# Girjoaba/simplex_method_gpu

Hardware: AMD Instinct MI355X
Metric: simplex iterations/sec on dense m=4096 n=16384 fp64; achieved HBM GB/s (higher is better)
Workload: dtype f64

## Files before the change

### include/simplex.h

```cpp
#ifndef SIMPLEX_MI355X_H
#define SIMPLEX_MI355X_H

#include <stdint.h>

#ifdef __cplusplus
extern "C" {
#endif

#define SPX_ABI_VERSION 8

#define SPX_STATUS_MAX_ITER       0
#define SPX_STATUS_OPTIMUM_FOUND  1
#define SPX_STATUS_UNBOUNDED      2
#define SPX_STATUS_THETA_OVERFLOW 3
#define SPX_STATUS_INFEASIBLE     4

#define SPX_OK             0
#define SPX_ERR_ARG       -1
#define SPX_ERR_HIP       -2
#define SPX_ERR_OOM       -3
#define SPX_ERR_RCCL      -4
#define SPX_ERR_STATE     -5
#define SPX_ERR_NO_DEVICE -6
#define SPX_ERR_SINGULAR  -7
// ... 143 lines not shown

int spx_solve(spx_ctx* ctx, int64_t max_iter, double* z, int64_t* b_ixs,
              double* x_b, int32_t* status, int64_t* pivots);

int spx_iterate(spx_ctx* ctx, int64_t k, int32_t* status, int64_t* pivots);

int spx_price(spx_ctx* ctx, int64_t* p, double* min_e, int32_t* optimal);
int spx_pivot(spx_ctx* ctx, int64_t* q, int32_t* status);

int spx_get_state(spx_ctx* ctx, double* x_b, int64_t* b_ixs, double* y,
                  double* c_b, double* binv_rowmajor, int32_t* status,
                  int64_t* pivots);

int spx_reduced_costs(spx_ctx* ctx, double* e);

int spx_objective(spx_ctx* ctx, double* z);

int spx_get_trace(spx_ctx* ctx, int64_t* p, int64_t* q, int64_t cap, int64_t* count);

int spx_get_weights(spx_ctx* ctx, double* w);

int spx_kernel_times(spx_ctx* ctx, double* price_ms, int64_t* price_launches,
                     double* update_ms, int64_t* update_launches);

int spx_pbox_vtb_times(spx_ctx* ctx, double* ms, int64_t* launches);

int spx_pbox_wexact_times(spx_ctx* ctx, double* ms, int64_t* launches);

int spx_ranging_times(spx_ctx* ctx, double ms[2], int64_t launches[2]);

int spx_pass_times(spx_ctx* ctx, double out[3], int64_t* passes);

#define SPX_PHASES 18
int spx_phase_times(spx_ctx* ctx, double out[SPX_PHASES]);

int spx_fold_times(spx_ctx* ctx, uint64_t* out, int64_t cap, int64_t* count);

int spx_wg_times(spx_ctx* ctx, uint64_t* out, int64_t cap, int64_t* count);

#define SPX_LOOP_FIELDS 7
int spx_loop_times(spx_ctx* ctx, double out[SPX_LOOP_FIELDS], int64_t* passes);

int spx_info(spx_ctx* ctx, int64_t* m, int64_t* n, int64_t* ld,
             int64_t* local_nonbasic, double* bytes_price, double* bytes_update);

#define SPX_CONFIG_FIELDS 17
int spx_config(spx_ctx* ctx, int32_t out[SPX_CONFIG_FIELDS]);

#define SPX_LOOP_LAYOUT_FIELDS 8
int spx_loop_layout(spx_ctx* ctx, int32_t out[SPX_LOOP_LAYOUT_FIELDS]);

int spx_ftran_cols(spx_ctx* ctx, int32_t* cols);

#define SPX_DISPATCH_FIELDS 12
int spx_dispatch_stats(spx_ctx* ctx, int64_t out[SPX_DISPATCH_FIELDS]);

int spx_prepare(spx_ctx* ctx);

int spx_shard_range(int64_t m, int64_t n, int32_t rank, int32_t nranks, int64_t out[4]);
int spx_minloc_merge(const double* vals, const int64_t* idx, int32_t count,
                     double* best_val, int64_t* best_idx);

const char* spx_last_error(void);
const char* spx_status_string(int32_t status);
int spx_abi_version(void);

#ifdef __cplusplus
}
#endif
#endif
```

### simplex_method_gpu_amd/__init__.py

```python
from __future__ import annotations

import ctypes
from dataclasses import dataclass
from enum import IntEnum
from typing import NamedTuple

import numpy as np

from ._lib import SimplexError, SpxOpts, check, load

__all__ = ["SolveStatus", "SolveResult", "Context", "solve", "read_lp", "comm_unique_id",
           "shard_range", "minloc_merge", "group_iterate", "group_sync", "check_ranks",
           "SimplexError", "FLAG_TIMING", "RATIO_REFERENCE", "RATIO_GUARDED", "RATIO_HARRIS",
           "PRICING_DANTZIG", "PRICING_DEVEX", "PRICING_STEEPEST", "ALGO_PRIMAL", "ALGO_DUAL",
           "DUAL_PRICING_DANTZIG", "DUAL_PRICING_STEEPEST", "FLAG_DUAL_STEEPEST",
           "DUAL_RATIO_TEXTBOOK", "DUAL_RATIO_LONG_STEP", "FLAG_DUAL_LONG_STEP", "ALGO_PRIMAL_BOX",
           "FLAG_PRIMAL_PHASE1", "PRIMAL_PRICING_DANTZIG", "PRIMAL_PRICING_STEEPEST", "FLAG_PRIMAL_STEEPEST",
           "PRIMAL_WEIGHTS_REFERENCE", "PRIMAL_WEIGHTS_EXACT", "FLAG_PRIMAL_EXACT_WEIGHTS",
           "CostRanging", "RhsRanging"]

FLAG_TIMING = 1
FLAG_STAMPS = 2
FLAG_GLOBAL_Y = 4
FLAG_ROW_SHARD = 8
# ... 457 lines not shown
        per = 4 * min(g, 4096) + 4 * min(gp, 4096) + 3
        out = np.zeros(2 * per, dtype=np.uint64)
        cnt = ctypes.c_int64()
        check(self._L.spx_wg_times(self._h, _ptr(out), out.size, ctypes.byref(cnt)))
        res = []
        for par in range(2):
            b = out[par * per: (par + 1) * per]
            nu, npr = 4 * min(g, 4096), 4 * min(gp, 4096)
            res.append({"ftran": b[:nu].reshape(-1, 4), "price": b[nu: nu + npr].reshape(-1, 4),
                        "tail": int(b[nu + npr]), "mark": int(b[nu + npr + 1]), "book": int(b[nu + npr + 2])})
        return res

    def fold_times(self):
        out = np.zeros(8 * 1024, dtype=np.uint64)
        cnt = ctypes.c_int64()
        check(self._L.spx_fold_times(self._h, _ptr(out), out.size, ctypes.byref(cnt)))
        return out.reshape(1024, 8)

    def phase_times(self):
        out = (ctypes.c_double * 18)()
        check(self._L.spx_phase_times(self._h, out))
        return {"price_body_us": out[0], "price_tail_us": out[1],
                "update_body_us": out[2], "update_tail_us": out[3],
                "tail_partials_us": out[4], "tail_sy_us": out[5], "tail_blocksum_us": out[6],
                "tail_bookkeeping_us": out[7], "update_prologue_us": out[9], "update_drain_us": out[10],
                "price_prologue_us": out[11], "price_drain_us": out[12],
                "upd_wg0_us": [round(out[13 + k], 2) for k in range(5)]}

    def loop_times(self):
        out, n = (ctypes.c_double * 7)(), ctypes.c_int64()
        check(self._L.spx_loop_times(self._h, out, ctypes.byref(n)))
        return {"loop_ms": out[0], "loop_passes": int(out[1]), "price_us": out[2], "ftran_us": out[3],
                "tail_us": out[4], "clock_passes": n.value, "fold_ms": out[5], "folds": int(out[6])}

    def pass_times(self):
        out, n = (ctypes.c_double * 3)(), ctypes.c_int64()
        check(self._L.spx_pass_times(self._h, out, ctypes.byref(n)))
        return {"price_ms": out[0], "price_minloc_ms": out[1], "update_ms": out[2], "passes": n.value}

    def info(self):
        m, n, ld, nb = ctypes.c_int64(), ctypes.c_int64(), ctypes.c_int64(), ctypes.c_int64()
        bp, bu = ctypes.c_double(), ctypes.c_double()
        check(self._L.spx_info(self._h, ctypes.byref(m), ctypes.byref(n), ctypes.byref(ld), ctypes.byref(nb),
                               ctypes.byref(bp), ctypes.byref(bu)))
        return {"m": m.value, "n": n.value, "ld": ld.value, "local_nonbasic": nb.value,
                "bytes_price": bp.value, "bytes_update": bu.value}


    def ftran_cols(self) -> int:
        v = ctypes.c_int32()
        check(self._L.spx_ftran_cols(self._h, ctypes.byref(v)))
        return v.value

    def dispatch_stats(self):
        out = (ctypes.c_int64 * 12)()
        check(self._L.spx_dispatch_stats(self._h, out))
        keys = ("eager_passes", "graph_launches", "graph_passes", "persistent_launches", "persistent_passes",
                "folds", "window_pos", "window", "persist_fallbacks", "graph_builds", "dw_anchors", "dw_carry")
        return dict(zip(keys, list(out)))

    def config(self):
        out = (ctypes.c_int32 * 17)()
        check(self._L.spx_config(self._h, out))
        keys = ("window", "price_block", "price_grid", "price_lds", "update_block", "update_rows", "update_grid",
                "graph_batch", "persistent", "loop_block", "tableau", "loop_grid", "defer_tail", "compact_fold",
                "ftran_rows_per_wave", "mbox_fused", "compact_price")
        cfg = dict(zip(keys, list(out)))
        cfg["dw_carry"] = self.dispatch_stats()["dw_carry"]
        cfg["dual_pricing"] = self._dual_pricing
        cfg["primal_pricing"] = self._primal_pricing
        cfg["dual_ratio"] = self._dual_ratio
        cfg["primal_weights"] = self._primal_weights
        return cfg

    def loop_layout(self):
        out = (ctypes.c_int32 * 8)()
        check(self._L.spx_loop_layout(self._h, out))
        keys = ("dual_price_lds", "dual_update_lds", "dual_se_update_lds", "dual_se_rho_lds", "pbox_price_lds",
                "pbox_update_lds", "pbox_se_lds_vecs", "slack_unit")
        return dict(zip(keys, list(out)))


def solve(A_cols, b, c, max_iter: int = (1 << 62), eps: float = 1e-7, device: int = -1,
          algorithm: int = ALGO_PRIMAL) -> SolveResult:
    with Context(A_cols, b, c, eps=eps, device=device, algorithm=algorithm) as ctx:
        return ctx.solve(max_iter)
```

### simplex_method_gpu_amd/_lib.py

```python
from __future__ import annotations

import ctypes
import os

_HERE = os.path.dirname(os.path.abspath(__file__))
LIB_PATH = os.environ.get("SPX_LIB") or os.path.join(_HERE, "libsimplex.so")

_d, _i32, _i64, _u64, _p = ctypes.c_double, ctypes.c_int32, ctypes.c_int64, ctypes.c_uint64, ctypes.c_void_p
_pp = ctypes.POINTER(ctypes.c_void_p)


class SpxOpts(ctypes.Structure):
    _fields_ = [
        ("eps", ctypes.c_double),
        ("device", ctypes.c_int32),
        ("rank", ctypes.c_int32),
        ("nranks", ctypes.c_int32),
        ("graph_batch", ctypes.c_int32),
        ("price_block", ctypes.c_int32),
        ("update_rows", ctypes.c_int32),
        ("price_grid", ctypes.c_int32),
        ("flags", ctypes.c_int32),
        ("update_block", ctypes.c_int32),
        ("window", ctypes.c_int32),
        ("ratio_test", ctypes.c_int32),
        ("refactor_every", ctypes.c_int32),
        ("piv_tol", ctypes.c_double),
        ("feas_tol", ctypes.c_double),
        ("pricing", ctypes.c_int32),
        ("loop_block", ctypes.c_int32),
        ("trace_cap", ctypes.c_int32),
        ("algorithm", ctypes.c_int32),
    ]


SIGNATURES = {
    "spx_default_opts": (None, [ctypes.POINTER(SpxOpts)]),
    "spx_create": (ctypes.c_int, [_pp, _i64, _i64, _p, _p, _p, ctypes.POINTER(SpxOpts)]),
    "spx_create_generated": (ctypes.c_int, [_pp, _i64, _i64, _u64, ctypes.POINTER(SpxOpts)]),
    "spx_destroy": (None, [_p]),
    "spx_comm_unique_id": (ctypes.c_int, [_p]),
    "spx_attach_comm": (ctypes.c_int, [_p, _p]),
    "spx_comm_info": (ctypes.c_int, [_p, _p, _p]),
    "spx_mbox_export": (ctypes.c_int, [_p, _p]),
    "spx_ftran_cols": (ctypes.c_int, [_p, _p]),
    "spx_mbox_attach": (ctypes.c_int, [_p, _p]),
    "spx_reset": (ctypes.c_int, [_p]),
    "spx_reinvert": (ctypes.c_int, [_p]),
    "spx_set_basis": (ctypes.c_int, [_p, _p]),
    "spx_set_algorithm": (ctypes.c_int, [_p, _i32]),
    "spx_set_rhs": (ctypes.c_int, [_p, _p]),
    "spx_set_bounds": (ctypes.c_int, [_p, _p]),
    "spx_get_bounds": (ctypes.c_int, [_p, _p]),
    "spx_set_bounds_lu": (ctypes.c_int, [_p, _p, _p]),
    "spx_get_bounds_lu": (ctypes.c_int, [_p, _p, _p]),
    "spx_get_primal": (ctypes.c_int, [_p, _p, _p]),
    "spx_set_dual_pricing": (ctypes.c_int, [_p, _i32]),
    "spx_get_dual_weights": (ctypes.c_int, [_p, _p]),
    "spx_set_dual_ratio": (ctypes.c_int, [_p, _i32]),
    "spx_set_primal_pricing": (ctypes.c_int, [_p, _i32]),
    "spx_get_primal_weights": (ctypes.c_int, [_p, _p]),
    "spx_get_dual_flips": (ctypes.c_int, [_p, _p]),
    "spx_set_cost": (ctypes.c_int, [_p, _p]),
    "spx_get_primal_flips": (ctypes.c_int, [_p, _p]),
    "spx_pbox_vtb_times": (ctypes.c_int, [_p, _p, _p]),
    "spx_set_primal_weight_init": (ctypes.c_int, [_p, _i32]),
    "spx_refresh_primal_weights": (ctypes.c_int, [_p]),
    "spx_pbox_wexact_times": (ctypes.c_int, [_p, _p, _p]),
    "spx_ranging_cost": (ctypes.c_int, [_p, _p, _p, _p, _p]),
    "spx_ranging_rhs": (ctypes.c_int, [_p, _p, _p, _p, _p]),
    "spx_ranging_times": (ctypes.c_int, [_p, _p, _p]),
    "spx_group_iterate": (ctypes.c_int, [_p, _i32, _i64, _p, _p]),
    "spx_group_sync": (ctypes.c_int, [_p, _i32]),
    "spx_solve": (ctypes.c_int, [_p, _i64, _p, _p, _p, _p, _p]),
    "spx_iterate": (ctypes.c_int, [_p, _i64, _p, _p]),
    "spx_price": (ctypes.c_int, [_p, _p, _p, _p]),
    "spx_pivot": (ctypes.c_int, [_p, _p, _p]),
    "spx_dispatch_stats": (ctypes.c_int, [_p, _p]),
    "spx_prepare": (ctypes.c_int, [_p]),
    "spx_get_trace": (ctypes.c_int, [_p, _p, _p, _i64, _p]),
    "spx_get_weights": (ctypes.c_int, [_p, _p]),
    "spx_get_state": (ctypes.c_int, [_p, _p, _p, _p, _p, _p, _p, _p]),
    "spx_reduced_costs": (ctypes.c_int, [_p, _p]),
    "spx_objective": (ctypes.c_int, [_p, _p]),
    "spx_kernel_times": (ctypes.c_int, [_p, _p, _p, _p, _p]),
    "spx_pass_times": (ctypes.c_int, [_p, _p, _p]),
    "spx_info": (ctypes.c_int, [_p, _p, _p, _p, _p, _p, _p]),
    "spx_config": (ctypes.c_int, [_p, _p]),
    "spx_loop_layout": (ctypes.c_int, [_p, _p]),
    "spx_phase_times": (ctypes.c_int, [_p, _p]),
    "spx_wg_times": (ctypes.c_int, [_p, _p, _i64, _p]),
    "spx_fold_times": (ctypes.c_int, [_p, _p, _i64, _p]),
    "spx_loop_times": (ctypes.c_int, [_p, _p, _p]),
    "spx_shard_range": (ctypes.c_int, [_i64, _i64, _i32, _i32, _p]),
    "spx_minloc_merge": (ctypes.c_int, [_p, _p, _i32, _p, _p]),
    "spx_last_error": (ctypes.c_char_p, []),
    "spx_status_string": (ctypes.c_char_p, [_i32]),
    "spx_abi_version": (ctypes.c_int, []),
# ... 35 lines not shown
```

### simplex_method_gpu_amd/csrc/spx_api.cpp

```cpp
#include <algorithm>
#include <cmath>
#include <cstdarg>
#include <cstdio>
#include <cstdlib>
#include <cstring>
#include <string>
#include <vector>

#include "spx_ctx.h"
#include "spx_tableau.h"

using namespace spx;
using namespace spx_host;

namespace {

thread_local std::string g_err;

}

int spx_host::fail(int code, const char* fmt, ...) {
    char buf[512];
    va_list ap;
    va_start(ap, fmt);
    vsnprintf(buf, sizeof(buf), fmt, ap);
    va_end(ap);
    g_err = buf;
    return code;
}

namespace {

int64_t round_up(int64_t v, int64_t a) { return (v + a - 1) / a * a; }

void shard_range(int64_t m, int64_t n, int r, int G, int64_t out[4]) {
    const int64_t ns = n - m;
    const int64_t sb = (ns + G - 1) / G, kb = (m + G - 1) / G;
    out[0] = std::min<int64_t>(ns, (int64_t)r * sb);
    out[1] = std::min<int64_t>(ns, (int64_t)(r + 1) * sb);
    out[2] = ns + std::min<int64_t>(m, (int64_t)r * kb);
    out[3] = ns + std::min<int64_t>(m, (int64_t)(r + 1) * kb);
}

}

extern "C" {

void spx_default_opts(spx_opts* o) {
    if (!o) return;
    std::memset(o, 0, sizeof(*o));
    o->eps = 1e-7;
    o->device = -1;
    o->rank = 0;
    o->nranks = 1;
    o->graph_batch = 0;
    o->ratio_test = SPX_RATIO_REFERENCE;
    o->refactor_every = 0;
    o->piv_tol = 1e-9;
    o->feas_tol = 1e-9;
    o->pricing = SPX_PRICING_DANTZIG;
}
// ... 863 lines not shown
        }
        SPX_TRY(x->alloc(&P.rlist, (size_t)x->L));
        SPX_TRY(x->alloc(&P.rmap, (size_t)x->L));
        SPX_TRY(x->alloc(&P.rleft, (size_t)x->L));
        SPX_TRY(x->alloc(&P.bc_n, BC_N_WORDS));
    }
    const UpdateCfg& uc = x->ucfg;
    const bool tail_ok = x->defer_ok || (x->use_comm && x->P.win && !x->P.split_tail && !x->P.row_shard &&
                                         !(x->opts.flags & SPX_FLAG_PRICE_TAIL));
    if (x->P.bc && tail_ok && !x->persist && !x->P.tab && uc.bc_entry && uc.rows == 1 &&
        uc.block == 512 && (x->pcfg.block == 512 || x->pcfg.block == 256) && !env_off("SPX_DEFER_TAIL")) {
        SPX_TRY(x->alloc(&x->P.trec, 1));
        HIP_TRY(hipMemset(x->P.trec, 0, sizeof(TailRec)));
        x->P.tail_parts = uc.grid;
        x->defer_tail = true;
    }
    x->se_fuse = x->P.steep && x->defer_tail && uc.bc_entry == 1 && uc.grid <= x->se_rows && !env_off("SPX_SE_FUSE");
    return SPX_OK;
}

int cprice_setup(spx_ctx* x) {
    Params& P = x->P;
    if (!(P.bc && !P.steep && x->opts.nranks == 1 && !x->use_comm && !x->persist && !P.row_shard &&
          (x->pcfg.wm == 1 || x->pcfg.wm == 2) && !env_on("SPX_DENSE_PRICE")))
        return SPX_OK;
    int64_t cap = std::min<int64_t>(4096, std::max<int64_t>(512, round_up((x->m + 3) / 4, 64)));
    if (const char* ev = std::getenv("SPX_CPRICE_CAP")) {
        const int64_t v = std::atoll(ev);
        if (v >= 1 && v < cap) cap = v;
    }
    void* d = nullptr;
    const size_t bytes = (size_t)(cap * x->n) * sizeof(double);
    if (hipMalloc(&d, bytes) != hipSuccess) {
        (void)hipGetLastError();
        return SPX_OK;
    }
    x->allocs.push_back(d);
    HIP_TRY(hipMemsetAsync(d, 0, bytes, x->stream));
    SPX_TRY(x->alloc(&P.dw, (size_t)x->n));
    SPX_TRY(x->alloc(&P.as_ord, (size_t)cap));
    SPX_TRY(x->alloc(&P.as_off, (size_t)65));
    PriceCfg& cc = x->ccfg;
    cc.block = (x->opts.price_block == 512 || x->opts.price_block == 1024) ? x->pcfg.block : 256;
    if (x->defer_tail && cc.block == 1024) cc.block = 512;
    cc.lds_y = false;
    cc.wm = 6;
    cc.tk = false;
    cc.lds_bytes = (size_t)(cc.block / 64) * sizeof(PricePartial) + 16 + (size_t)round_up(cap, 2) * 16;
    x->dcfg = x->pcfg;
    x->dcfg.dw = true;
    int per_cu = 0, per_cu_d = 0;
    HIP_TRY(price_prepare(cc, &per_cu));
    HIP_TRY(price_prepare(x->dcfg, &per_cu_d));
    const int waves = cc.block / 64;
    cc.grid = (int)std::max<int64_t>(1, std::min<int64_t>({(x->max_local_cols + waves - 1) / waves,
                                                           (int64_t)x->cus * std::max(per_cu, 1), P.price_cap}));
    if (x->opts.price_grid > 0) cc.grid = (int)std::min<int64_t>(x->opts.price_grid, P.price_cap);
    P.as_ld = cap;
    P.as_cap = (int32_t)cap;
    P.AS = static_cast<double*>(d);
    x->cp_ok = x->cp_now = true;
    x->dwc.period = P.cfold ? spx_host::dw_period_from(std::getenv("SPX_DW_ANCHOR")) : 1;
    return SPX_OK;
}

int create_tail(spx_ctx* x) {
    SPX_TRY(do_reset(x));
    if (x->algo == SPX_ALGO_DUAL) return dual_setup(x);
    if (x->algo == SPX_ALGO_PRIMAL_BOX) return pbox_setup(x);
    if (!x->use_comm && !x->persist) SPX_TRY(build_graphs(x));
    return SPX_OK;
}

}

namespace spx_host {

bool env_on(const char* name) {
    const char* env = std::getenv(name);
    return env && env[0] == '1';
}
bool env_off(const char* name) {
    const char* env = std::getenv(name);
    return env && env[0] == '0';
}
size_t env_bytes(const char* name) {
    const char* env = std::getenv(name);
    const long long v = env ? std::atoll(env) : 0;
    return v >= 1 ? (size_t)v : 0;
}

int clear_tickets(spx_ctx* x) {
    HIP_TRY(hipMemsetAsync(x->P.tickets, 0, TICKET_WORDS * sizeof(uint32_t), x->stream));
    return SPX_OK;
}

int pass_events(spx_ctx* x, hipEvent_t* p0, hipEvent_t* p1, hipEvent_t* u0, hipEvent_t* u1) {
    auto grow = [](std::vector<hipEvent_t>& pool, size_t want) -> int {
        while (pool.size() < want) {
            hipEvent_t e;
            HIP_TRY(hipEventCreate(&e));
            pool.push_back(e);
        }
        return SPX_OK;
    };
    SPX_TRY(grow(x->ev_price, 2 * (x->n_price + 1)));
// ... 793 lines not shown
    out[10] = h[19] * 0.01;
    out[11] = h[22] * 0.01;
    out[12] = h[23] * 0.01;
    for (int k = 0; k < 5; ++k) out[13 + k] = h[24 + k] * 0.01;
    out[0] = h[1] * 0.01;
    out[1] = h[2] * 0.01;
    out[2] = h[5] * 0.01;
    out[3] = h[6] * 0.01;
    return reset_stamps(x);
}

int spx_info(spx_ctx* x, int64_t* m, int64_t* n, int64_t* ld, int64_t* local_nb, double* bp, double* bu) {
    if (!x) return fail(SPX_ERR_ARG, "ctx is NULL");
    SPX_TRY(read_state(x));
    if (m) *m = x->m;
    if (n) *n = x->n;
    if (ld) *ld = x->L;
    if (local_nb) *local_nb = x->st_host->nb_count;
    int64_t streamed = x->st_host->nb_count;
    if (x->P.slack_unit) {
        std::vector<int64_t> bix((size_t)x->m);
        HIP_TRY(hipMemcpy(bix.data(), x->P.b_ixs, (size_t)x->m * sizeof(int64_t), hipMemcpyDeviceToHost));
        int64_t basic_slacks = 0;
        for (int64_t j : bix) basic_slacks += (j >= x->P.k_lo && j < x->P.k_hi) ? 1 : 0;
        streamed -= (x->P.k_hi - x->P.k_lo) - basic_slacks;
    }
    if (bp) *bp = 8.0 * (double)(x->m + 1) * (double)streamed;
    if (bp && x->cp_ok && x->cp_now && x->P.win > 2) {
        const double kw = (double)x->P.win;
        const double per_col = 8.0 * ((double)x->s_list + 2.0 + 0.5 * (kw - 1.0) + 1.0);
        const double compact = per_col * (double)x->st_host->nb_count;
        *bp = spx_host::dw_mean_price_bytes(*bp, compact, x->P.win, x->dwc.period);
    }
    int32_t cols = 0;
    SPX_TRY(spx_ftran_cols(x, &cols));
    const double md = (double)x->m;
    double fold = (x->P.bc && x->P.cfold) ? 8.0 * md * (3.0 * cols + x->P.win) : 16.0 * md * md;
    if (x->cp_now && dw_carries(x) && x->P.win > 2)
        fold += spx_host::dw_carry_bytes(x->n, x->P.win) * (x->dwc.period > 0 ? 1.0 - 1.0 / x->dwc.period : 1.0);
    if (bu) *bu = x->P.win ? 8.0 * md * (double)cols + fold / (x->P.win - 1) : 16.0 * md * md;
    return SPX_OK;
}

int spx_ftran_cols(spx_ctx* x, int32_t* cols) {
    if (!x || !cols) return fail(SPX_ERR_ARG, "NULL argument");
    *cols = (int32_t)x->m;
    if (x->P.win && x->P.bc) {
        HIP_TRY(hipStreamSynchronize(x->stream));
        HIP_TRY(hipMemcpy(cols, x->P.bc_n, sizeof(int32_t), hipMemcpyDeviceToHost));
    }
    return SPX_OK;
}

int spx_config(spx_ctx* x, int32_t out[SPX_CONFIG_FIELDS]) {
    if (!x || !out) return fail(SPX_ERR_ARG, "NULL argument");
    out[0] = x->P.win;
    out[1] = x->pcfg.block;
    out[2] = x->pcfg.grid;
    out[3] = !x->pcfg.lds_y ? 0 : (x->pcfg.wm == 1 ? 2 : 1);
    out[4] = x->ucfg.block;
    out[5] = x->ucfg.rows;
    out[6] = x->ucfg.grid;
    out[7] = x->batch;
    out[8] = x->persist ? 1 : 0;
    out[9] = x->persist ? x->lcfg.block : 0;
    out[10] = x->P.tab;
    out[11] = x->persist ? x->lcfg.grid : 0;
    out[12] = x->defer_tail ? 1 : 0;
    out[13] = (x->P.bc && x->P.cfold) ? 1 : 0;
    out[14] = (x->P.bc && x->ucfg.rows == 1 && x->ucfg.bc_entry) ? x->ucfg.bc_entry : 0;
    out[15] = (x->mbox_ready && x->mbox_fused) ? 1 : 0;
    out[16] = (x->cp_ok && x->cp_now) ? 1 : 0;
    return SPX_OK;
}

int spx_shard_range(int64_t m, int64_t n, int32_t rank, int32_t nranks, int64_t out[4]) {
    if (!out || m <= 0 || n < m || nranks < 1 || rank < 0 || rank >= nranks)
        return fail(SPX_ERR_ARG, "bad shard arguments");
    shard_range(m, n, rank, nranks, out);
    return SPX_OK;
}

int spx_minloc_merge(const double* vals, const int64_t* idx, int32_t count, double* best_val, int64_t* best_idx) {
    if ((count > 0 && (!vals || !idx)) || !best_val || !best_idx) return fail(SPX_ERR_ARG, "NULL argument");
    ArgMinEntry b{INFINITY, INT64_MAX};
    for (int32_t g = 0; g < count; ++g)
        if (argmin_better(vals[g], idx[g], b.val, b.idx)) b = ArgMinEntry{vals[g], idx[g]};
    *best_val = b.val;
    *best_idx = b.idx;
    return SPX_OK;
}

}
```

### simplex_method_gpu_amd/csrc/spx_device.h

```cpp
#pragma once
#include <stdint.h>

namespace spx {

enum : int32_t {
    ST_RUNNING = 0,
    ST_OPTIMAL = 1,
    ST_UNBOUNDED = 2,
    ST_BREAKDOWN = 3,
    ST_INFEASIBLE = 4,
    ST_WINDOW_FULL = 16,
    ST_HANDOFF_TIMEOUT = 17,
    ST_CPRICE_STATE = 18
};

struct alignas(16) ArgMinEntry {
    double val;
    int64_t idx;
};

struct alignas(16) PricePartial {
    double val;
    int64_t idx;
    double w;
// ... 122 lines not shown
    int32_t price_dyn;
    int32_t tk_shards;
    int32_t win;
    int32_t pad_w;
    double* U;
    double* Wt;
    double* Qrows;
    double* Urows;
    double* SY;
    double* xw;
    int32_t ratio;
    int32_t devex;
    double piv_tol;
    double feas_tol;
    double* W;
    double* dvx_e;
    int32_t steep;
    int32_t se_parts;
    double* se_v;
    double* se_cg;
    double* se_part;
    int32_t defer_price;
    int32_t price_grid;
    int32_t defer_tail;
    int32_t tail_parts;
    TailRec* trec;
    int32_t tab;
    int32_t tab_slack;
    double* T;
    double* dw;
    int32_t* tab_list;
    int32_t* tab_cnt;
    int64_t* trace;
    int64_t trace_cap;
    uint32_t* arrive;
    uint64_t* const* mbox_peer;
    uint64_t* mbox;
    uint32_t* mbox_seq;
    int32_t mbox_rank;
    int32_t mbox_fused;
    int32_t slack_unit;
    int32_t bc_lds;
    double* bc;
    double* bc1;
    int32_t cfold;
    int32_t se_fused;
    int32_t* rlist;
    int32_t* rmap;
    int32_t* rleft;
    int32_t* bc_n;
    double* AS;
    int64_t as_ld;
    int32_t as_cap;
    int32_t pad_as;
    int32_t* as_ord;
    int32_t* as_off;
};

__host__ __device__ inline double* bc_buf(const Params& P, int sel) { return sel ? P.bc1 : P.bc; }
constexpr int BC_N_WORDS = 8;

__device__ __forceinline__ void record_pivot(const Params& P, int64_t it, int64_t p, int64_t q) {
    if (P.trace && it < P.trace_cap) {
        P.trace[2 * it] = p;
        P.trace[2 * it + 1] = q;
    }
}

__host__ __device__ inline bool no_entering(const Params& P, double val, int64_t p) {
    return p == INT64_MAX || (P.devex ? !(val < INFINITY) : val >= -P.eps);
}

enum : int32_t { RATIO_REFERENCE = 0, RATIO_GUARDED = 1, RATIO_HARRIS = 2 };

__host__ __device__ inline double ratio_key(const Params& P, double xb, double a) {
    if (!(a > P.piv_tol)) return INFINITY;
    if (P.ratio == RATIO_REFERENCE) return xb / a;
    const double xc = xb > 0.0 ? xb : 0.0;
    return P.ratio == RATIO_HARRIS ? (xc + P.feas_tol) / a : xc / a;
}

__host__ __device__ inline bool owns_col(const Params& P, int64_t j) {
    return (j < P.ns) ? (j >= P.s_lo && j < P.s_hi) : (j >= P.k_lo && j < P.k_hi);
}

}
```

### simplex_method_gpu_amd/csrc/spx_price.hip

```cpp
#include <hip/hip_runtime.h>
#include <hip/hip_ext.h>
#include <math.h>

#include "spx_device.h"
#include "spx_common.h"
#include "spx_handoff.h"
#include "spx_kernels.h"
#include "spx_tabdev.h"

namespace spx {

#ifndef SPX_LDS_BATCH
#define SPX_LDS_BATCH 4
#endif
#ifndef SPX_PRICE_CH
#define SPX_PRICE_CH 8
#endif
#ifndef SPX_PRICE_DEEP
#define SPX_PRICE_DEEP 1
#endif
#ifndef SPX_SE_LDS_BATCH
#define SPX_SE_LDS_BATCH 2
#endif
#ifndef SPX_PRICE_DEEP_SE
#define SPX_PRICE_DEEP_SE 2
#endif
#ifndef SPX_PRICE_DYN_PCT
#define SPX_PRICE_DYN_PCT 85
#endif
#ifndef SPX_PRICE_PIPE
#define SPX_PRICE_PIPE 1
#endif

template <int WAVES>
__device__ __forceinline__ int best_wave(const PricePartial* red) {
    double bv = red[0].val;
    int64_t bi = red[0].idx;
    int bk = 0;
#pragma unroll
    for (int i = 1; i < WAVES; ++i) {
        const double v = red[i].val;
        const int64_t x = red[i].idx;
        if (argmin_better(v, x, bv, bi)) {
            bv = v;
            bi = x;
            bk = i;
        }
    }
    return bk;
}

template <int BLOCK, bool LDS_Y, int WM, bool TK = false, bool DW = false>
__global__ __launch_bounds__(BLOCK) void k_price(Params P) {
    DevState* st = P.st;
    constexpr int WAVES = BLOCK / 64;
    constexpr bool WIN = WM != 0;
    constexpr bool CP = WM == 6;
    static_assert(!DW || WM == 1 || WM == 2, "dw is stored by the dense window passes");
    constexpr bool LDS_R = WM == 1 || WM == 4;
    constexpr bool SE = WM == 4 || WM == 5;
    constexpr bool LDS_V = WM == 4;
    const int tid = threadIdx.x;
    const int lane = tid & 63;
    const int wave = __builtin_amdgcn_readfirstlane(tid >> 6);
    const int idx0 = blockIdx.x * WAVES + wave;
    int64_t j0 = P.nb_list[idx0 < P.n ? idx0 : P.n - 1];
    const unsigned long long t_pw0 = P.stamps ? rtime() : 0ull;
    constexpr bool PAIR = BLOCK == 256;
    constexpr bool DT = WM != 0 && WM != 3;
    TailRec R{};
    if constexpr (DT) R = *(P.defer_tail ? P.trec : reinterpret_cast<const TailRec*>(P.zeros));
    int cp_S = 0, cp_ld = 64, cp_sel = 0, cp_dw = 0;
    if constexpr (CP) {
        cp_S = P.bc_n[0];
        cp_ld = P.bc_n[1];
        cp_sel = P.bc_n[2];
        cp_dw = P.bc_n[5];
    }
    typedef unsigned int u32x4 __attribute__((ext_vector_type(4)));
    constexpr int SW = (int)(sizeof(DevState) / 16);
    u32x4 sw[SW];
#pragma unroll
    for (int i = 0; i < SW; ++i) sw[i] = reinterpret_cast<const u32x4*>(st)[i];
    UpdPartial w0 = upd_empty(), w1 = upd_empty();
    if constexpr (DT) {
        const int tp = P.tail_parts > 0 ? P.tail_parts : 1;
        w0 = upd_fetch<true>(P, tid < tp ? tid : tp - 1);
        if constexpr (PAIR) w1 = upd_fetch<true>(P, tid + BLOCK < tp ? tid + BLOCK : tp - 1);
    }
    __builtin_amdgcn_sched_barrier(0);
#pragma unroll
    for (int i = 0; i < SW; ++i) asm volatile("" ::"v"(sw[i]));
    const DevState S = __builtin_bit_cast(DevState, sw);
    int64_t s_iter = S.iter, s_q = S.q, s_leave = S.leave;
    double s_aq = S.aq, s_sy = S.s_y, s_wp = S.wp;
    int32_t s_nb = S.nb_count, s_nw = S.nw;
    bool fresh = false;
    int32_t pk_a = -1, pk_b = -1;
    int64_t pv_a = 0, pv_b = 0;
    constexpr int CH = (BLOCK <= 512 && WM != 3) ? SPX_PRICE_CH : 8;
    constexpr int LB = (WM == 4 && SPX_SE_LDS_BATCH > 0) ? SPX_SE_LDS_BATCH : SPX_LDS_BATCH;
    constexpr bool DEEP2 = SPX_PRICE_DEEP && SPX_PRICE_PIPE && BLOCK <= 512 && CH == 8 &&
                           (WM == 1 || (SPX_PRICE_DEEP_SE == 2 && WM == 4));
    constexpr bool DEEP = DEEP2 || (SPX_PRICE_DEEP_SE && SPX_PRICE_PIPE && WM == 4 && BLOCK <= 512 && CH == 8);
    dbl2 vd0[DEEP ? CH : 1], vd1[DEEP2 ? CH : 1];
    int64_t jdeep = -1;
    __shared__ TailRec s_rec;
    __shared__ UpdPartial s_tp;
    if (DT && P.defer_tail) {
        fresh = R.fresh != 0;
// ... 326 lines not shown
                    P.W[j] = wt;
                }
                key = (e < -P.eps) ? -(e * e) / wt : INFINITY;
            }
            if (argmin_better(key, j, best, bj)) { best = key; bj = j; bw = w; be = e; }
        }
        wave_price_min(best, bj, bw, be);
    } else if constexpr (CP) {
        double* cf = reinterpret_cast<double*>(smem + WAVES * sizeof(PricePartial) + 16);
        const int capp = (P.as_cap + 1) & ~1;
        int* cpos = reinterpret_cast<int*>(cf + capp);
        int* crow = cpos + capp;
        __shared__ int c_off[65];
        const int Sn = pend ? cp_S : 0;
        {
            const double* bq = bc_buf(P, cp_sel) + qq * (int64_t)cp_ld;
            for (int i = tid; i < Sn; i += BLOCK) {
                const int c = P.as_ord[i];
                cpos[i] = c;
                crow[i] = P.rlist[c];
                cf[i] = bq[c];
            }
            if (tid < 65) c_off[tid] = pend ? P.as_off[tid] : 0;
        }
        const bool unitq = pend && P.rmap[qq] < 0 && lane == (int)((qq >> 1) & 63);
        __syncthreads();
        const int i0 = min(max(c_off[lane], 0), Sn), i1 = min(max(c_off[lane + 1], i0), Sn);
        const int64_t ald = P.as_ld;
        constexpr int KR = 8;
        double rc0[KR], rc1[KR];
        int rp[KR];
        int iR = i0;
        bool qrem = unitq;
#pragma unroll
        for (int u = 0; u < KR; ++u) {
            const bool takeq = qrem && (iR >= i1 || crow[iR] > (int)qq);
            double cv = 0.0;
            int par = 0;
            rp[u] = 0;
            if (takeq) {
                rp[u] = -1;
                cv = 1.0;
                par = (int)(qq & 1);
                qrem = false;
            } else if (iR < i1) {
                rp[u] = cpos[iR];
                cv = cf[iR];
                par = crow[iR] & 1;
                ++iR;
            }
            rc0[u] = par ? 0.0 : cv;
            rc1[u] = par ? cv : 0.0;
        }
        double av[KR], wv = 0.0, dv = 0.0, aqj = 0.0;
        auto request = [&](int64_t jj, double (&xa)[KR], double& xw, double& xd, double& xq) {
            const double* as = P.AS + jj * ald;
            const double* aq = P.A + jj * L + qq;
            xw = (pend && lane < tau) ? P.Wt[jj * KW + lane] : 0.0;
            xd = lane == 0 ? P.dw[jj] : 0.0;
#pragma unroll
            for (int u = 0; u < KR; ++u) xa[u] = *(rp[u] < 0 ? aq : as + rp[u]);
            xq = qrem ? *aq : 0.0;
        };
        const int ilast = nlist > 0 ? nlist - 1 : 0;
        int64_t jn = nbl(idx0 + stride < nlist ? idx0 + stride : ilast);
        if (idx0 < nlist) request(j0, av, wv, dv, aqj);
        int64_t jc = j0;
        for (int idx = idx0; idx < nlist; idx += stride) {
            const int64_t j = jc;
            const double* as = P.AS + j * ald;
            const int64_t jn2 = nbl(idx + 2 * stride < nlist ? idx + 2 * stride : ilast);
            double avn[KR], wvn = 0.0, dvn = 0.0, aqn = 0.0;
            const bool more = idx + stride < nlist;
            if (more) request(jn, avn, wvn, dvn, aqn);
            double b0 = 0.0, b1 = 0.0;
#pragma unroll
            for (int u = 0; u < KR; ++u) {
                b0 = fma(av[u], rc0[u], b0);
                b1 = fma(av[u], rc1[u], b1);
            }
            bool qdone = !qrem;
            auto unit_term = [&]() {
                if (qq & 1) b1 = fma(aqj, 1.0, b1);
                else b0 = fma(aqj, 1.0, b0);
                qdone = true;
            };
            for (int i = iR; i < i1; ++i) {
                const int r = crow[i];
                if (!qdone && r > (int)qq) unit_term();
                const double a = as[cpos[i]];
                if (r & 1) b1 = fma(a, cf[i], b1);
                else b0 = fma(a, cf[i], b0);
            }
            if (!qdone) unit_term();
            double sa = fma(syl, wv, dv);
            double wn = fma(uq, wv, b0 + b1);
            wave_sum2(sa, wn);
            if (pend && lane == 0) P.Wt[j * KW + tau] = wn;
            const double e = pend ? fma(syp, wn, sa) : sa;
            consider(j, e, wn, 0.0);
            if (more) {
#pragma unroll
                for (int u = 0; u < KR; ++u) av[u] = avn[u];
                wv = wvn;
                dv = dvn;
                aqj = aqn;
            }
            jc = jn;
            jn = jn2;
        }
    } else {
    auto unit_col = [&](int64_t jj) { return P.slack_unit && jj >= P.ns; };
    bool have = pre && !unit_col(j0);
    int idx_next = 0;
    for (int idx = idx0; idx < nlist; idx = idx_next) {
        const bool first = idx == idx0;
        if constexpr (DYN) {
            if (tkc && idx < s_lim && idx + stride >= s_lim) {
                uint32_t t = 0;
                if (lane == 0) t = __hip_atomic_fetch_add(tkc, 1u, __ATOMIC_RELAXED, __HIP_MEMORY_SCOPE_AGENT);
                tk_pend = t;
            }
        }
        const int64_t j = first ? j0 : nbl(idx);
        const dbl2* __restrict__ col = reinterpret_cast<const dbl2*>(P.A + j * L);
        double wv = 0.0;
        if (WIN && pend && lane < tau) wv = P.Wt[j * KW + lane];
        double a0 = 0.0, a1 = 0.0, b0 = 0.0, b1 = 0.0, d0 = 0.0, d1 = 0.0;
        int64_t k = lane;
        const bool unit = unit_col(j);
        const bool pipe = SPX_PRICE_PIPE && BLOCK <= 512 && have && (L2 & 511) == 0 && L2 > CH * 64;
        auto run_pipe = [&](auto pend_t) {
            constexpr bool PD = decltype(pend_t)::value;
            auto consume = [&](const dbl2* vv, int nb8, int64_t kb) {
#pragma unroll
                for (int h = 0; h < 8; h += LB) {
                    if (h >= nb8) break;
                    dbl2 w[LB], r[LB], x[LB];
#pragma unroll
                    for (int u = 0; u < LB; ++u) {
                        w[u] = Y(kb + lane + (h + u) * 64);
                        if constexpr (PD) r[u] = Rw(kb + lane + (h + u) * 64);
                        if constexpr (PD && SE) x[u] = Vw(kb + lane + (h + u) * 64);
                    }
#pragma unroll
                    for (int u = 0; u < LB; ++u) {
                        a0 = fma(vv[h + u].x, w[u].x, a0);
                        a1 = fma(vv[h + u].y, w[u].y, a1);
                        if constexpr (PD) {
                            b0 = fma(vv[h + u].x, r[u].x, b0);
                            b1 = fma(vv[h + u].y, r[u].y, b1);
                        }
                        if constexpr (PD && SE) {
                            d0 = fma(vv[h + u].x, x[u].x, d0);
                            d1 = fma(vv[h + u].y, x[u].y, d1);
                        }
                    }
                }
            };
            int64_t kb = CH * 64;
            dbl2 vc[8];
            if (DEEP2 && first && deep_hit) {
                kb = 2 * CH * 64;
// ... 356 lines not shown
        }
    }
    if (WIN && P.nin > 1) {
        double* wo = reinterpret_cast<double*>(P.price_out + 1);
        if (tid < KW)
            wo[tid] = (t.idx == INT64_MAX || tid >= nw) ? 0.0 : (tid == tau ? t.w : P.Wt[t.idx * KW + tid]);
    }
    stamp_tail(slot, t_tail, win);
}

template <int BLOCK, bool LDS_Y, int WM, bool TK = false, bool DW = false>
static hipError_t launch_price_t(const Params& P, int grid, size_t lds, hipStream_t s, hipEvent_t e0,
                                 hipEvent_t e1) {
    if (e0 || e1) {
        hipExtLaunchKernelGGL((k_price<BLOCK, LDS_Y, WM, TK, DW>), dim3(grid), dim3(BLOCK), (uint32_t)lds, s, e0, e1, 0, P);
    } else {
        hipLaunchKernelGGL((k_price<BLOCK, LDS_Y, WM, TK, DW>), dim3(grid), dim3(BLOCK), lds, s, P);
    }
    return hipGetLastError();
}

template <int BLOCK, bool LDS_Y, int WM, bool TK = false, bool DW = false>
static hipError_t prep_price_t(size_t lds, int* blocks_per_cu) {
    hipError_t e = hipSuccess;
    if (lds > 65536) {
        e = hipFuncSetAttribute(reinterpret_cast<const void*>(&k_price<BLOCK, LDS_Y, WM, TK, DW>),
                                hipFuncAttributeMaxDynamicSharedMemorySize, (int)lds);
        if (e != hipSuccess) return e;
    }
    return hipOccupancyMaxActiveBlocksPerMultiprocessor(blocks_per_cu, k_price<BLOCK, LDS_Y, WM, TK, DW>, BLOCK, lds);
}

template <int BLOCK>
static hipError_t price_dispatch(const PriceCfg& c, const Params* P, hipStream_t s, hipEvent_t e0, hipEvent_t e1,
                                 int* blocks_per_cu) {
#define SPX_PV(LY, WM)                                                                  \
    return P ? launch_price_t<BLOCK, LY, WM>(*P, c.grid, c.lds_bytes, s, e0, e1)        \
             : prep_price_t<BLOCK, LY, WM>(c.lds_bytes, blocks_per_cu)
#define SPX_PVD(LY, WM, TK)                                                                    \
    return P ? launch_price_t<BLOCK, LY, WM, TK, true>(*P, c.grid, c.lds_bytes, s, e0, e1)     \
             : prep_price_t<BLOCK, LY, WM, TK, true>(c.lds_bytes, blocks_per_cu)
    if (c.dw) {
        if (c.wm == 1 && c.lds_y) {
            if (c.tk) SPX_PVD(true, 1, true);
            SPX_PVD(true, 1, false);
        }
        if (c.wm == 2) {
            if (c.lds_y) SPX_PVD(true, 2, false);
            SPX_PVD(false, 2, false);
        }
        return hipErrorInvalidValue;
    }
    if (c.wm == 6) SPX_PV(false, 6);
    if (c.wm == 0) {
        if (c.lds_y) SPX_PV(true, 0);
        SPX_PV(false, 0);
    }
    if (c.wm == 1 && c.lds_y) {
        if (c.tk) return P ? launch_price_t<BLOCK, true, 1, true>(*P, c.grid, c.lds_bytes, s, e0, e1)
                           : prep_price_t<BLOCK, true, 1, true>(c.lds_bytes, blocks_per_cu);
        SPX_PV(true, 1);
    }
    if (c.wm == 2) {
        if (c.lds_y) SPX_PV(true, 2);
        SPX_PV(false, 2);
    }
    if (c.wm == 3) SPX_PV(false, 3);
    if (c.wm == 4 && c.lds_y) SPX_PV(true, 4);
    if (c.wm == 5) {
        if (c.lds_y) SPX_PV(true, 5);
        SPX_PV(false, 5);
    }
#undef SPX_PV
#undef SPX_PVD
    return hipErrorInvalidValue;
}

__global__ __launch_bounds__(256) void k_dw_basic(Params P) {
    const int lane = threadIdx.x & 63;
    const int64_t L2 = P.L >> 1;
    const double* y = P.st->y_buf ? P.y1 : P.y0;
    const dbl2* y2 = reinterpret_cast<const dbl2*>(y);
    for (int64_t i = ((int64_t)blockIdx.x * blockDim.x + threadIdx.x) >> 6; i < P.m;
         i += ((int64_t)gridDim.x * blockDim.x) >> 6) {
        const int64_t j = P.b_ixs[i];
        if ((uint64_t)j >= (uint64_t)P.n) continue;
        double s;
        if (P.slack_unit && j >= P.ns) {
            s = y[j - P.ns] - P.c[j];
        } else {
            const dbl2* col = reinterpret_cast<const dbl2*>(P.A + j * P.L);
            double a0 = 0.0, a1 = 0.0;
            for (int64_t k = lane; k < L2; k += 64) {
                const dbl2 v = col[k], w = y2[k];
                a0 = fma(v.x, w.x, a0);
                a1 = fma(v.y, w.y, a1);
            }
            s = wave_sum(a0 + a1) - P.c[j];
        }
        if (lane == 0) P.dw[j] = s;
    }
}

hipError_t launch_dw_basic(const Params& P, hipStream_t s) {
    const int64_t want = (P.m + 3) / 4;
    hipLaunchKernelGGL(k_dw_basic, dim3((unsigned)(want < 1024 ? want : 1024)), dim3(256), 0, s, P);
// ... 23 lines not shown
```

Before: 31260.

## Stage compact-price row segments in LDS with coalesced multi-column prefetch

Adds a new pricing mode (wm=7) for the compact-row pricing path. Each wave loads a contiguous chunk of up to 512 rows of a column into a per-wave LDS slot with coalesced lane-strided reads and keeps several columns in flight. The sparse row gathers then read from LDS instead of issuing scattered global loads. LDS usage is sized per wave, and the row limit steps down in tiers if occupancy would drop. It becomes the default when the row cap allows, at the cost of more LDS, registers and extra wave barriers.

```diff
diff --git a/include/simplex.h b/include/simplex.h
--- a/include/simplex.h
+++ b/include/simplex.h
@@ -219,6 +219,8 @@
 
 int spx_ftran_cols(spx_ctx* ctx, int32_t* cols);
 
+int spx_cprice_rows(spx_ctx* ctx, int32_t out[2]);
+
 #define SPX_DISPATCH_FIELDS 12
 int spx_dispatch_stats(spx_ctx* ctx, int64_t out[SPX_DISPATCH_FIELDS]);
 
diff --git a/simplex_method_gpu_amd/__init__.py b/simplex_method_gpu_amd/__init__.py
--- a/simplex_method_gpu_amd/__init__.py
+++ b/simplex_method_gpu_amd/__init__.py
@@ -533,6 +533,11 @@
         check(self._L.spx_ftran_cols(self._h, ctypes.byref(v)))
         return v.value
 
+    def cprice_rows(self):
+        out = (ctypes.c_int32 * 2)()
+        check(self._L.spx_cprice_rows(self._h, out))
+        return {"rows": out[0], "slot_bytes": out[1]}
+
     def dispatch_stats(self):
         out = (ctypes.c_int64 * 12)()
         check(self._L.spx_dispatch_stats(self._h, out))
diff --git a/simplex_method_gpu_amd/_lib.py b/simplex_method_gpu_amd/_lib.py
--- a/simplex_method_gpu_amd/_lib.py
+++ b/simplex_method_gpu_amd/_lib.py
@@ -44,6 +44,7 @@
     "spx_comm_info": (ctypes.c_int, [_p, _p, _p]),
     "spx_mbox_export": (ctypes.c_int, [_p, _p]),
     "spx_ftran_cols": (ctypes.c_int, [_p, _p]),
+    "spx_cprice_rows": (ctypes.c_int, [_p, _p]),
     "spx_mbox_attach": (ctypes.c_int, [_p, _p]),
     "spx_reset": (ctypes.c_int, [_p]),
     "spx_reinvert": (ctypes.c_int, [_p]),
diff --git a/simplex_method_gpu_amd/csrc/spx_api.cpp b/simplex_method_gpu_amd/csrc/spx_api.cpp
--- a/simplex_method_gpu_amd/csrc/spx_api.cpp
+++ b/simplex_method_gpu_amd/csrc/spx_api.cpp
@@ -7,6 +7,7 @@
 #include <string>
 #include <vector>
 
+#include "spx_cprows.h"
 #include "spx_ctx.h"
 #include "spx_tableau.h"
 
@@ -976,6 +977,16 @@
     int per_cu = 0, per_cu_d = 0;
     HIP_TRY(price_prepare(cc, &per_cu));
     HIP_TRY(price_prepare(x->dcfg, &per_cu_d));
+    const size_t lds_base = cc.lds_bytes;
+    P.cp_rows = spx_cprows::limit_from(std::getenv("SPX_CPRICE_ROWS"), cap);
+    for (;;) {
+        int with_slots = per_cu;
+        cc.lds_bytes = lds_base + spx_cprows::lds_bytes(cc.block / 64, P.cp_rows);
+        cc.wm = P.cp_rows > 0 ? 7 : 6;
+        if (P.cp_rows > 0) HIP_TRY(price_prepare(cc, &with_slots));
+        if (P.cp_rows == 0 || with_slots >= per_cu) break;
+        P.cp_rows = spx_cprows::tier_below(P.cp_rows);
+    }
     const int waves = cc.block / 64;
     cc.grid = (int)std::max<int64_t>(1, std::min<int64_t>({(x->max_local_cols + waves - 1) / waves,
                                                            (int64_t)x->cus * std::max(per_cu, 1), P.price_cap}));
@@ -1875,6 +1886,13 @@
     return SPX_OK;
 }
 
+int spx_cprice_rows(spx_ctx* x, int32_t out[2]) {
+    if (!x || !out) return fail(SPX_ERR_ARG, "NULL argument");
+    out[0] = x->cp_ok ? x->P.cp_rows : 0;
+    out[1] = x->cp_ok ? (int32_t)(spx_cprows::slot_doubles(x->P.cp_rows) * sizeof(double)) : 0;
+    return SPX_OK;
+}
+
 int spx_config(spx_ctx* x, int32_t out[SPX_CONFIG_FIELDS]) {
     if (!x || !out) return fail(SPX_ERR_ARG, "NULL argument");
     out[0] = x->P.win;
diff --git a/simplex_method_gpu_amd/csrc/spx_cprows.h b/simplex_method_gpu_amd/csrc/spx_cprows.h
--- /dev/null
+++ b/simplex_method_gpu_amd/csrc/spx_cprows.h
@@ -0,0 +1,39 @@
+#pragma once
+#include <algorithm>
+#include <cstddef>
+#include <cstdint>
+#include <cstdlib>
+
+#if defined(__HIPCC__)
+#define SPX_CPROWS_HD __host__ __device__
+#else
+#define SPX_CPROWS_HD
+#endif
+
+namespace spx_cprows {
+
+constexpr int ROWS_MAX = 512;
+constexpr int ROWS_DEFAULT = 512;
+
+SPX_CPROWS_HD constexpr int chunks(int S, int limit) {
+    return (S <= 0 || S > limit || S > ROWS_MAX) ? 0 : (S <= 128 ? 2 : (S <= 256 ? 4 : 8));
+}
+SPX_CPROWS_HD constexpr int depth(int nc) { return (nc == 2 || nc == 4) ? 4 : 2; }
+SPX_CPROWS_HD constexpr int slot_doubles(int limit) { return limit > 0 ? 64 * chunks(limit, limit) + 2 : 0; }
+SPX_CPROWS_HD constexpr size_t lds_bytes(int waves, int limit) {
+    return (size_t)waves * (size_t)slot_doubles(limit) * sizeof(double);
+}
+
+SPX_CPROWS_HD constexpr int tier_below(int limit) { return limit > 256 ? 256 : (limit > 128 ? 128 : 0); }
+
+inline int32_t limit_from(const char* env, int64_t cap) {
+    long v = ROWS_DEFAULT;
+    if (env && *env) {
+        char* end = nullptr;
+        const long t = std::strtol(env, &end, 10);
+        if (end != env && t >= 0) v = t;
+    }
+    return (int32_t)std::max<int64_t>(0, std::min<int64_t>({(int64_t)v, cap, (int64_t)ROWS_MAX}));
+}
+
+}
diff --git a/simplex_method_gpu_amd/csrc/spx_device.h b/simplex_method_gpu_amd/csrc/spx_device.h
--- a/simplex_method_gpu_amd/csrc/spx_device.h
+++ b/simplex_method_gpu_amd/csrc/spx_device.h
@@ -198,7 +198,7 @@
     double* AS;
     int64_t as_ld;
     int32_t as_cap;
-    int32_t pad_as;
+    int32_t cp_rows;
     int32_t* as_ord;
     int32_t* as_off;
 };
diff --git a/simplex_method_gpu_amd/csrc/spx_price.hip b/simplex_method_gpu_amd/csrc/spx_price.hip
--- a/simplex_method_gpu_amd/csrc/spx_price.hip
+++ b/simplex_method_gpu_amd/csrc/spx_price.hip
@@ -4,6 +4,7 @@
 
 #include "spx_device.h"
 #include "spx_common.h"
+#include "spx_cprows.h"
 #include "spx_handoff.h"
 #include "spx_kernels.h"
 #include "spx_tabdev.h"
@@ -55,7 +56,8 @@
     DevState* st = P.st;
     constexpr int WAVES = BLOCK / 64;
     constexpr bool WIN = WM != 0;
-    constexpr bool CP = WM == 6;
+    constexpr bool CP = WM == 6 || WM == 7;
+    constexpr bool CPR = WM == 7;
     static_assert(!DW || WM == 1 || WM == 2, "dw is stored by the dense window passes");
     constexpr bool LDS_R = WM == 1 || WM == 4;
     constexpr bool SE = WM == 4 || WM == 5;
@@ -488,63 +490,187 @@
             rc0[u] = par ? 0.0 : cv;
             rc1[u] = par ? cv : 0.0;
         }
-        double av[KR], wv = 0.0, dv = 0.0, aqj = 0.0;
-        auto request = [&](int64_t jj, double (&xa)[KR], double& xw, double& xd, double& xq) {
-            const double* as = P.AS + jj * ald;
-            const double* aq = P.A + jj * L + qq;
-            xw = (pend && lane < tau) ? P.Wt[jj * KW + lane] : 0.0;
-            xd = lane == 0 ? P.dw[jj] : 0.0;
-#pragma unroll
-            for (int u = 0; u < KR; ++u) xa[u] = *(rp[u] < 0 ? aq : as + rp[u]);
-            xq = qrem ? *aq : 0.0;
-        };
-        const int ilast = nlist > 0 ? nlist - 1 : 0;
-        int64_t jn = nbl(idx0 + stride < nlist ? idx0 + stride : ilast);
-        if (idx0 < nlist) request(j0, av, wv, dv, aqj);
-        int64_t jc = j0;
-        for (int idx = idx0; idx < nlist; idx += stride) {
-            const int64_t j = jc;
-            const double* as = P.AS + j * ald;
-            const int64_t jn2 = nbl(idx + 2 * stride < nlist ? idx + 2 * stride : ilast);
-            double avn[KR], wvn = 0.0, dvn = 0.0, aqn = 0.0;
-            const bool more = idx + stride < nlist;
-            if (more) request(jn, avn, wvn, dvn, aqn);
-            double b0 = 0.0, b1 = 0.0;
-#pragma unroll
-            for (int u = 0; u < KR; ++u) {
-                b0 = fma(av[u], rc0[u], b0);
-                b1 = fma(av[u], rc1[u], b1);
-            }
-            bool qdone = !qrem;
-            auto unit_term = [&]() {
-                if (qq & 1) b1 = fma(aqj, 1.0, b1);
-                else b0 = fma(aqj, 1.0, b0);
-                qdone = true;
+        if constexpr (CPR) {
+            auto consider_plain = [&](int64_t j, double e, double wn) {
+                if (argmin_better(e, j, best, bj)) { best = e; bj = j; bw = wn; be = e; }
             };
-            for (int i = iR; i < i1; ++i) {
-                const int r = crow[i];
-                if (!qdone && r > (int)qq) unit_term();
-                const double a = as[cpos[i]];
-                if (r & 1) b1 = fma(a, cf[i], b1);
-                else b0 = fma(a, cf[i], b0);
-            }
-            if (!qdone) unit_term();
-            double sa = fma(syl, wv, dv);
-            double wn = fma(uq, wv, b0 + b1);
-            wave_sum2(sa, wn);
-            if (pend && lane == 0) P.Wt[j * KW + tau] = wn;
-            const double e = pend ? fma(syp, wn, sa) : sa;
-            consider(j, e, wn, 0.0);
-            if (more) {
-#pragma unroll
-                for (int u = 0; u < KR; ++u) av[u] = avn[u];
-                wv = wvn;
-                dv = dvn;
-                aqj = aqn;
-            }
-            jc = jn;
-            jn = jn2;
-        }
+            auto run_rows = [&](auto nc_t, auto dv_t) {
+                constexpr int NC = decltype(nc_t)::value;
+                constexpr bool DV = decltype(dv_t)::value;
+                constexpr int D = spx_cprows::depth(NC);
+                constexpr int MASK = 64 * NC - 1;
+                if (idx0 >= nlist) return;
+                double* slot = reinterpret_cast<double*>(crow + capp) + wave * spx_cprows::slot_doubles(P.cp_rows);
+                const int lim = min(cp_S, (int)ald);
+                int pu[KR];
+#pragma unroll
+                for (int u = 0; u < KR; ++u) pu[u] = rp[u] < 0 ? 64 * NC : (rp[u] & MASK);
+                const bool has_w = pend && lane < tau;
+                const int wl = has_w ? lane : 0;
+                constexpr int R = D - 1;
+                double xr[R][NC], xw[R], xo[R];
+                int jr[R];
+                auto request = [&](int64_t jj, double (&r)[NC], double& w, double& o) {
+                    const double* as = P.AS + jj * ald;
+                    w = P.Wt[jj * KW + wl];
+                    o = *(lane == 0 ? P.dw + jj : P.A + jj * L + qq);
+#pragma unroll
+                    for (int t = 0; t < NC; ++t) {
+                        const int i = lane + 64 * t;
+                        r[t] = as[i < lim ? i : 0];
+                    }
+                };
+                const int ilast = nlist - 1;
+                auto list64 = [&](int k0) -> int {
+                    const int64_t i = (int64_t)idx0 + ((int64_t)k0 + lane) * stride;
+                    return (int)nbl(i < nlist ? (int)i : ilast);
+                };
+                int jl = 0, idx = idx0, k = 0;
+                auto step = [&](auto d_t) {
+                    constexpr int d = decltype(d_t)::value;
+                    const int64_t j = jr[d];
+                    const double wv = has_w ? xw[d] : 0.0;
+                    const double dv = lane == 0 ? xo[d] : 0.0;
+                    const double aqj = unitq ? (lane == 0 ? readlane_d(xo[d], 1) : xo[d]) : 0.0;
+                    __builtin_amdgcn_wave_barrier();
+#pragma unroll
+                    for (int t = 0; t < NC; ++t) slot[lane + 64 * t] = xr[d][t];
+                    if (unitq) slot[64 * NC] = aqj;
+                    __builtin_amdgcn_wave_barrier();
+                    jr[d] = __builtin_amdgcn_readlane(jl, min(k + R, 63));
+                    request(jr[d], xr[d], xw[d], xo[d]);
+                    double av[KR];
+#pragma unroll
+                    for (int u = 0; u < KR; ++u) av[u] = slot[pu[u]];
+                    double b0 = 0.0, b1 = 0.0;
+#pragma unroll
+                    for (int u = 0; u < KR; ++u) {
+                        b0 = fma(av[u], rc0[u], b0);
+                        b1 = fma(av[u], rc1[u], b1);
+                    }
+                    bool qdone = !qrem;
+                    auto unit_term = [&]() {
+                        if (qq & 1) b1 = fma(aqj, 1.0, b1);
+                        else b0 = fma(aqj, 1.0, b0);
+                        qdone = true;
+                    };
+                    for (int i = iR; i < i1; ++i) {
+                        const int r = crow[i];
+                        if (!qdone && r > (int)qq) unit_term();
+                        const double a = slot[cpos[i] & MASK];
+                        if (r & 1) b1 = fma(a, cf[i], b1);
+                        else b0 = fma(a, cf[i], b0);
+                    }
+                    if (!qdone) unit_term();
+                    __builtin_amdgcn_wave_barrier();
+                    double sa = fma(syl, wv, dv);
+                    double wn = fma(uq, wv, b0 + b1);
+                    wave_sum2(sa, wn);
+                    if (pend && lane == 0) P.Wt[j * KW + tau] = wn;
+                    const double e_j = pend ? fma(syp, wn, sa) : sa;
+                    if constexpr (DV) consider(j, e_j, wn, 0.0);
+                    else consider_plain(j, e_j, wn);
+                    idx += stride;
+                    ++k;
+                };
+                int k0 = 0;
+                while (idx < nlist) {
+                    jl = list64(k0);
+                    k0 += 64;
+#pragma unroll
+                    for (int d = 0; d < R; ++d) {
+                        jr[d] = __builtin_amdgcn_readlane(jl, d);
+                        request(jr[d], xr[d], xw[d], xo[d]);
+                    }
+                    const int64_t left = ((int64_t)nlist - idx + stride - 1) / stride;
+                    const int ng = (int)(left < 64 ? left : 64);
+                    k = 0;
+                    while (k + R <= ng) {
+                        step(std::integral_constant<int, 0>());
+                        if constexpr (R == 3) {
+                            step(std::integral_constant<int, 1>());
+                            step(std::integral_constant<int, 2>());
+                        } else {
+                            static_assert(R == 1, "one or three columns requested ahead");
+                        }
+                    }
+                    if constexpr (R == 3) {
+                        const int rem = ng - k;
+                        if (rem >= 1) step(std::integral_constant<int, 0>());
+                        if (rem >= 2) step(std::integral_constant<int, 1>());
+                    }
+                }
+            };
+            const int cp_nc = spx_cprows::chunks(cp_S, P.cp_rows);
+            const bool cp_dv = P.devex != 0;
+            if (cp_nc == 2 && !cp_dv) run_rows(std::integral_constant<int, 2>(), std::false_type());
+            else if (cp_nc == 4 && !cp_dv) run_rows(std::integral_constant<int, 4>(), std::false_type());
+            else if (cp_nc == 8 && !cp_dv) run_rows(std::integral_constant<int, 8>(), std::false_type());
+            else if (cp_nc == 2) run_rows(std::integral_constant<int, 2>(), std::true_type());
+            else if (cp_nc == 4) run_rows(std::integral_constant<int, 4>(), std::true_type());
+            else if (cp_nc == 8) run_rows(std::integral_constant<int, 8>(), std::true_type());
+            if (cp_nc != 0) goto cp_priced;
+        }
+        {
+            double av[KR], wv = 0.0, dv = 0.0, aqj = 0.0;
+            auto request = [&](int64_t jj, double (&xa)[KR], double& xw, double& xd, double& xq) {
+                const double* as = P.AS + jj * ald;
+                const double* aq = P.A + jj * L + qq;
+                xw = (pend && lane < tau) ? P.Wt[jj * KW + lane] : 0.0;
+                xd = lane == 0 ? P.dw[jj] : 0.0;
+#pragma unroll
+                for (int u = 0; u < KR; ++u) xa[u] = *(rp[u] < 0 ? aq : as + rp[u]);
+                xq = qrem ? *aq : 0.0;
+            };
+            const int ilast = nlist > 0 ? nlist - 1 : 0;
+            int64_t jn = nbl(idx0 + stride < nlist ? idx0 + stride : ilast);
+            if (idx0 < nlist) request(j0, av, wv, dv, aqj);
+            int64_t jc = j0;
+            for (int idx = idx0; idx < nlist; idx += stride) {
+                const int64_t j = jc;
+                const double* as = P.AS + j * ald;
+                const int64_t jn2 = nbl(idx + 2 * stride < nlist ? idx + 2 * stride : ilast);
+                double avn[KR], wvn = 0.0, dvn = 0.0, aqn = 0.0;
+                const bool more = idx + stride < nlist;
+                if (more) request(jn, avn, wvn, dvn, aqn);
+                double b0 = 0.0, b1 = 0.0;
+#pragma unroll
+                for (int u = 0; u < KR; ++u) {
+                    b0 = fma(av[u], rc0[u], b0);
+                    b1 = fma(av[u], rc1[u], b1);
+                }
+                bool qdone = !qrem;
+                auto unit_term = [&]() {
+                    if (qq & 1) b1 = fma(aqj, 1.0, b1);
+                    else b0 = fma(aqj, 1.0, b0);
+                    qdone = true;
+                };
+                for (int i = iR; i < i1; ++i) {
+                    const int r = crow[i];
+                    if (!qdone && r > (int)qq) unit_term();
+                    const double a = as[cpos[i]];
+                    if (r & 1) b1 = fma(a, cf[i], b1);
+                    else b0 = fma(a, cf[i], b0);
+                }
+                if (!qdone) unit_term();
+                double sa = fma(syl, wv, dv);
+                double wn = fma(uq, wv, b0 + b1);
+                wave_sum2(sa, wn);
+                if (pend && lane == 0) P.Wt[j * KW + tau] = wn;
+                const double e = pend ? fma(syp, wn, sa) : sa;
+                consider(j, e, wn, 0.0);
+                if (more) {
+#pragma unroll
+                    for (int u = 0; u < KR; ++u) av[u] = avn[u];
+                    wv = wvn;
+                    dv = dvn;
+                    aqj = aqn;
+                }
+                jc = jn;
+                jn = jn2;
+            }
+        }
+        [[maybe_unused]] cp_priced:;
     } else {
     auto unit_col = [&](int64_t jj) { return P.slack_unit && jj >= P.ns; };
     bool have = pre && !unit_col(j0);
@@ -1007,6 +1133,7 @@
         return hipErrorInvalidValue;
     }
     if (c.wm == 6) SPX_PV(false, 6);
+    if (c.wm == 7) SPX_PV(false, 7);
     if (c.wm == 0) {
         if (c.lds_y) SPX_PV(true, 0);
         SPX_PV(false, 0);
```

After: 32320, median of 6. +3.4%, better.
